# samkatt/fba-pomdp

Measured on AMD Instinct MI355X. Metric: simulated env steps/sec (belief+rollout), higher is better.
Workload: dtype f64

## Files before the change

fba_pomdp_amd/csrc/fba_engine.hip:

```cpp
#include <hip/hip_runtime.h>

#include <algorithm>
#include <cmath>
#include <cstdarg>
#include <cstdio>
#include <cstdlib>
#include <cstring>
#include <string>
#include <map>
#include <memory>
#include <vector>

#include "fba_belief_factors.h"
#include "fba_launch_plan.h"
#include "fba_snapshot_format.h"

using namespace fba;

namespace {

thread_local std::string g_create_error;

struct EventPair {
    hipEvent_t a, b;
// ... 1151 lines not shown
{
    std::vector<unsigned long long> h((size_t)n);
    hipError_t e = hipMemcpy(h.data(), dev, h.size() * sizeof(unsigned long long), hipMemcpyDeviceToHost);
    if (e != hipSuccess) {
        *rc = fail(c, FBA_EHIP, "counter download failed: %s", hipGetErrorString(e));
        return 0;
    }
    uint64_t s = 0;
    for (auto v : h) s += v;
    return s;
}


struct CreateSwitches {
    bool double_buffer, node_visits, wide_hash, dense_particles;
    bool no_etiger, tiger_gather, no_compact;
    int hist_multi;
    bool hist_lockstep;
    bool tree_records, rows_hbm, stride_full;
    bool is_multi_min_set;
    int is_multi_min;
    int scratch_slots, node_bound;
    int node_words;
};
CreateSwitches read_create_switches()
{
    const auto number = [](const char* v, int unset) { return v ? std::atoi(v) : unset; };
    const auto says   = [](const char* v, const char* word) { return v && !std::strcmp(v, word); };
    const auto at_least = [](const char* v, int least) { return v ? std::max(least, std::atoi(v)) : 0; };
    CreateSwitches s{};
    s.double_buffer   = std::getenv("FBA_DOUBLE_BUFFER") != nullptr;
    s.node_visits     = std::getenv("FBA_NODE_VISITS") != nullptr;
    s.wide_hash       = std::getenv("FBA_WIDE_HASH") != nullptr;
    s.dense_particles = std::getenv("FBA_DENSE_PARTICLES") != nullptr;
    s.no_etiger       = number(std::getenv("FBA_NO_ETIGER"), 0) != 0;
    s.tiger_gather    = number(std::getenv("FBA_TIGER_GATHER"), 0) != 0;
    s.no_compact      = number(std::getenv("FBA_NO_COMPACT"), 0) != 0;
    const char* multi = std::getenv("FBA_HIST_MULTI");
    s.hist_multi      = multi ? (std::atoi(multi) != 0 ? 2 : 1) : 0;
    s.hist_lockstep   = number(std::getenv("FBA_HIST_LOCKSTEP"), 1) != 0;
    s.tree_records    = says(std::getenv("FBA_HIST_TREE"), "records");
    s.rows_hbm        = says(std::getenv("FBA_HIST_ROWS"), "hbm");
    s.stride_full     = says(std::getenv("FBA_HIST_STRIDE"), "full");
    const char* multi_min = std::getenv("FBA_IS_MULTI_MIN");
    s.is_multi_min_set = multi_min != nullptr;
    s.is_multi_min     = multi_min ? std::max(1, std::atoi(multi_min)) : IS_MAX_CHUNKS * 256 + 1;
    s.scratch_slots   = at_least(std::getenv("FBA_SCRATCH_SLOTS"), 1);
    s.node_bound      = at_least(std::getenv("FBA_NODE_BOUND"), 2);
    s.node_words      = number(std::getenv("FBA_NODE_WORDS"), 0);
    return s;
}

int check_arguments(const fba_config& cfg)
{
    if (cfg.sims < 1 && cfg.planner == FBA_PLANNER_POUCT) return fail(nullptr, FBA_EINVAL, "cannot initiate POUCT with %d simulations, must be greater than 0", cfg.sims);
    if (cfg.horizon <= 0) return fail(nullptr, FBA_EINVAL, "cannot initiate POUCT with %d horizon, must be greater than 0", cfg.horizon);
    if (cfg.horizon > 255) return fail(nullptr, FBA_EINVAL, "horizon %d exceeds the 255 steps a stream address holds", cfg.horizon);
    if (cfg.particles < 1) return fail(nullptr, FBA_EINVAL, "cannot initiate belief with n = %d", cfg.particles);
    if (cfg.discount <= 0 || cfg.discount > 1) return fail(nullptr, FBA_EINVAL, "discount must be in (0, 1]");
    if (cfg.runs < 1 || cfg.episodes < 1) return fail(nullptr, FBA_EINVAL, "runs and episodes must be >= 1");
    if (cfg.episodes > 65535) return fail(nullptr, FBA_EINVAL, "episodes %d exceeds the 65535 a stream address holds", cfg.episodes);
    if (cfg.model == FBA_MODEL_POMDP && cfg.episodes != 1) return fail(nullptr, FBA_EINVAL, "planning runs have exactly one episode per run");
    int ndev = 0;
    if (hipGetDeviceCount(&ndev) != hipSuccess || ndev <= 0) return fail(nullptr, FBA_ENODEVICE, "no HIP device visible: libfba_hip has no CPU path");
    if (cfg.device < 0 || cfg.device >= ndev) return fail(nullptr, FBA_EINVAL, "device %d out of range (%d visible)", cfg.device, ndev);
    return FBA_OK;
}

bool has_fully_connected_prior(const fba_config& cfg)
{
    return cfg.model == FBA_MODEL_BA_FACTORED && (dom_is_ftiger(cfg.domain) || is_ca(cfg.domain) || is_sys(cfg.domain)) &&
           !(is_ca(cfg.domain) && cfg.structure_prior == FBA_SP_FULLY_CONNECTED);
// ... 320 lines not shown
    }
    P.search_budget = (P.hist && P.hist != 3 && cfg.search_budget > 0) ? cfg.search_budget : 0;
    const size_t per_particle_aux = (P.hist && P.belief == FBA_BELIEF_REJECTION) ? 0 : (size_t)(2 * 8 + 8 + 4 * (MAXINC + 1));
    t.per_slot = (size_t)P.N * (per_particle_aux + ((P.reinvig || P.cheat) ? 4 : (P.incub ? 6 : (P.hist ? 1 : 2))) * (size_t)P.Cs * 4) +
                 (t.bkt_lines ? t.bkt_lines * 128 : (size_t)D.max_nodes * D.node_words * 4 + (size_t)t.hcap * t.hash_entry) + 1024;
    return FBA_OK;
}

int slot_count(const fba_config& cfg, const TreePlan& t, size_t budget)
{
    if (cfg.slots > 0) return cfg.slots;
    return std::min((int)std::min<size_t>(std::max<size_t>(budget / t.per_slot, 1), 32768), cfg.runs);
}

bool weighted_filters(const Problem& P) { return P.belief == FBA_BELIEF_IMPORTANCE || P.incub; }

int plan_filters(fba_ctx* c, const CreateSwitches& sw)
{
    const Problem& P = c->P;
    DeviceState& D = c->D;
    D.single_rec      = P.hist && !sw.double_buffer ? 1 : 0;
    D.ab_rows_hbm = sw.rows_hbm ? 1 : 0; D.ab_hist_multi = sw.hist_multi; D.ab_no_etiger = sw.no_etiger ? 1 : 0; D.ab_tiger_gather = sw.tiger_gather ? 1 : 0;
    D.ab_lockstep = sw.hist_lockstep ? 1 : 0;
    D.side_w = 1 + (P.model == FBA_MODEL_BA_FACTORED ? c->fdesc.FS + c->fdesc.FO : (P.model == FBA_MODEL_BA_TABLE ? 2 : 0));
    if (P.hist) D.side_w = 2;
    D.is_multi    = weighted_filters(P) && P.N >= sw.is_multi_min;
    D.ctot_stride = (P.N + 255) / 256 + 2;
    if (P.mh) {
        if (D.is_multi) return fail(c, FBA_EINVAL, "mh-within-gibbs belief: at most %d particles per slot", IS_MAX_CHUNKS * 256);
        if (c->fdesc.nvar > MH_MAXVAR) return fail(c, FBA_EINVAL, "mh beliefs: at most %d structure words per particle", MH_MAXVAR);
        size_t words = (size_t)3 * P.Cs + (size_t)P.S * P.A * P.S + (size_t)P.A * P.S * P.O + 2;
        words += 2 * ((size_t)(P.horizon + 1) * P.S + P.S) + (size_t)P.episodes * (P.horizon + 1) + 2 * (size_t)P.horizon + 2;
        D.mh_scratch_words = (int32_t)((words + 3) & ~(size_t)3);
    }
    if (P.cheat && D.is_multi) return fail(c, FBA_EINVAL, "cheating-reinvigoration belief: at most %d particles per slot", IS_MAX_CHUNKS * 256);
    return FBA_OK;
}

bool compact_filters_ok(const fba_ctx* c, const CreateSwitches& sw)
{
    const Problem& P = c->P;
    return c->cfg.domain == FBA_DOM_TIGER_EPISODIC && P.belief == FBA_BELIEF_REJECTION && !P.reinvig && !P.incub && !P.cheat && !P.nested &&
           !P.point && run_steps(c->cfg) <= 32767 && !sw.dense_particles && !sw.no_compact && P.search_budget <= 0 &&
           kernel_name(update_plan(P, c->D).filter) == K_REJECT_TIGER_ONCE && search_plan(P, c->D).kernel == SEARCH_READS_COMPACT;
}

// ... 2049 lines not shown
```

fba_pomdp_amd/csrc/fba_launch_plan.h:

```cpp
#pragma once

#include "fba_kernels.h"

namespace fba {

__host__ __device__ __forceinline__ bool root_children_in_lds(const Problem& P, const DeviceState& D)
{
    return P.A * P.O <= ROOT_CHILDREN && D.max_nodes <= 32767;
}
constexpr int ET_NODE_WORDS = 9;
__host__ __device__ __forceinline__ size_t search_lds_words(const Problem& P, const DeviceState& D, bool stage, bool etiger)
{
    const int depth_cap = P.max_depth > 0 ? P.max_depth : 1;
    if (etiger)
        return (size_t)((depth_cap + 1) / 2) * SEARCH_BLOCK + (stage ? (size_t)P.Cs * SEARCH_BLOCK : 0) + (size_t)2 * ET_NODE_WORDS * SEARCH_BLOCK;
    return (size_t)depth_cap * SEARCH_BLOCK * 2 + (stage ? (size_t)P.Cs * SEARCH_BLOCK : 0) +
           (root_children_in_lds(P, D) ? (size_t)P.A * P.O * SEARCH_BLOCK / 2 : 0);
}
constexpr int HIST_TREES = SEARCH_BLOCK / HIST_QUAD;
constexpr int H2_WAVES = 4;
__host__ __device__ __forceinline__ size_t h2_shared_bytes(const Problem& P, bool lrows)
{
    const int K = hist_row_width(P.hist_row);
    return lrows ? (size_t)P.hist_rid_bytes + (size_t)P.hist_distinct * K * sizeof(float) : (size_t)4 * HistLayout(P.gw_N, P.gw_G, 4).ostride * sizeof(float);
// ... 42 lines not shown
}
constexpr uint32_t importance_key(bool reg, int tiger_table, bool hist, bool wlds) { return kernel_key(K_IMPORTANCE, reg, tiger_table, hist, wlds); }
constexpr bool tiger_filter_in_lds(uint32_t key)
{
    return kernel_name(key) == K_REJECT_TIGER_LDS || kernel_name(key) == K_REJECT_TIGER_ONCE || kernel_name(key) == K_REJECT_TIGER_ONCE_GATHER;
}
constexpr bool reads_packed_tiger(uint32_t key)
{
    return key == search_key(true, 4, false, 2, FBA_MODEL_BA_TABLE) || key == SEARCH_READS_COMPACT || key == reject_key(false, 2, 0, 512) ||
           tiger_filter_in_lds(key) || key == importance_key(false, 2, false, false) || key == importance_key(false, 2, false, true);
}
constexpr bool reads_packed_ftiger(uint32_t key, int fs = 4)
{
    return key == reject_key(false, 0, fs, REJECT_BLOCK, true) || key == search_key(true, 4, false, 0, FBA_MODEL_BA_FACTORED, fs, false, true, false) ||
           key == search_key(true, 4, false, 0, FBA_MODEL_BA_FACTORED, fs, false, true, true) || (fs > 2 && reads_packed_ftiger(key, fs - 1));
}
constexpr bool updates_history_records(uint32_t key)
{
    return kernel_name(key) == K_REJECT_HIST || kernel_name(key) == K_REJECT_TAB_HIST || kernel_name(key) == K_IS_MULTI_TAB_STEP ||
           kernel_name(key) == K_IS_MULTI_CA_STEP || key == importance_key(false, 0, true, false) || key == importance_key(false, 0, true, true) ||
           (kernel_name(key) == K_IS_MULTI_STEP && (key >> 12 & 63));
}

struct SearchPlan {
    uint32_t kernel;
    int block, slots_per_block;
    size_t lds;
    int raise_lds;
    bool order_first;
    int grid(int slots) const { return (slots + slots_per_block - 1) / slots_per_block; }
};
inline SearchPlan search_plan(const Problem& P, const DeviceState& D)
{
    SearchPlan pl{0, SEARCH_BLOCK, SEARCH_BLOCK, 0, 0, false};
    const int depth_cap = P.max_depth > 0 ? P.max_depth : 1;
    if (P.hist == 3) {
        pl.kernel = kernel_key(K_SEARCH_CA_HIST, 4);
        pl.lds    = ca_hist_search_lds(P);
        return pl;
    }
    if (P.hist) {
        const int K = hist_row_width(P.hist_row);
        pl.slots_per_block = HIST_TREES;
        if (!D.bkt) {
            pl.kernel = kernel_key(K_SEARCH_HIST, K);
            pl.lds = (size_t)depth_cap * HIST_TREES * (sizeof(double) + sizeof(int32_t) + sizeof(float) + sizeof(int32_t)) + (size_t)P.Cs * HIST_TREES * sizeof(float);
            return pl;
        }
        const bool tab = P.hist == 2, flat = P.belief == FBA_BELIEF_REJECTION;
        const bool lrows = !tab && P.hist_lds != nullptr && !D.ab_rows_hbm;
        const size_t shared = tab ? 0 : h2_shared_bytes(P, lrows);
        int nw = H2_WAVES;
        while (nw > 1 && shared + (size_t)nw * h2_wave_bytes(P) > 64 * 1024) nw >>= 1;
        pl.lds = shared + (size_t)nw * h2_wave_bytes(P);
        pl.block = 64 * nw;
        pl.slots_per_block = HIST_TREES * nw;
        pl.raise_lds = pl.lds > 64 * 1024 ? (int)pl.lds : 0;
        pl.order_first = D.ab_lockstep != 0;
        pl.kernel = tab ? kernel_key(K_SEARCH_TABHIST, flat) : kernel_key(flat ? K_HIST2_FLAT_SEARCH : K_SEARCH_HIST2, K, lrows);
        return pl;
    }
    const bool stage = P.model != FBA_MODEL_POMDP && P.Cs <= SEARCH_STAGE_WORDS;
    const bool plain_tree  = P.planner == FBA_PLANNER_POUCT && !D.hash;
    const bool tiger_table = tiger_table_model(P) && stage && plain_tree;
    const bool tiger_pomdp = P.model == FBA_MODEL_POMDP && dom_is_tiger(P.domain) && plain_tree;
    const int fs           = ftiger_features(P);
    const bool ftiger      = fs >= 2 && fs <= 4 && plain_tree;
    const bool et = !D.ab_no_etiger && etiger_ok(P, D) && (tiger_table || tiger_pomdp || (ftiger && P.ft_packed));
    pl.lds = search_lds_words(P, D, stage, et) * sizeof(uint32_t);
    if (P.model == FBA_MODEL_BA_FACTORED && !ftiger)
        pl.lds = ((pl.lds + 15) & ~(size_t)15) + (((size_t)P.fd_bytes + 15) & ~(size_t)15);
    if (tiger_table) pl.kernel = search_key(true, 4, false, P.packed ? 2 : 1, FBA_MODEL_BA_TABLE, 0, false, false, et);
    else if (tiger_pomdp) pl.kernel = search_key(false, 4, false, 0, FBA_MODEL_POMDP, 0, true, false, et);
    else if (ftiger) pl.kernel = search_key(stage || P.ft_packed, 4, false, 0, FBA_MODEL_BA_FACTORED, fs, false, P.ft_packed != 0, et);
    else {
        const int amax  = P.A <= 4 ? 4 : (P.A <= 8 ? 8 : (P.A <= 16 ? 16 : 24));
        const int model = amax < 24 && (P.model == FBA_MODEL_BA_FACTORED || P.model == FBA_MODEL_BA_TABLE) ? P.model : FBA_MODEL_POMDP;
        pl.kernel = search_key(stage && model != FBA_MODEL_POMDP, amax, P.dirichlet_regular && model != FBA_MODEL_POMDP, 0, model);
    }
    return pl;
}

struct LaunchStep {
    uint32_t kernel;
    int block;
    int rows;
    int per_group;
    size_t lds;
    int raise_lds;
    int arg;
    bool chunked;
    bool shadow;
    dim3 grid(int slots) const { return rows ? dim3(rows, slots) : dim3((slots + per_group - 1) / per_group); }
};
struct LaunchPlan {
    LaunchStep step[12];
    int n = 0;
    uint32_t filter = 0;
    LaunchStep& add(uint32_t kernel, int block = 256, int rows = 0, int per_group = 1, size_t lds = 0, int arg = 0)
    {
        step[n] = LaunchStep{kernel, block, rows, per_group, lds, 0, arg, false, false};
        return step[n++];
// ... 117 lines not shown
```

fba_pomdp_amd/csrc/fba_search.hip:

```cpp
#include <algorithm>
#include <cstdio>
#include <cstdlib>
#include <cstring>

#include "fba_kernels_common.h"

namespace fba {

__device__ __forceinline__ int et_reward_code(double r) { return r == -1.0 ? 0 : (r == 10.0 ? 1 : 2); }
__device__ __forceinline__ double et_reward(int code) { return code == 0 ? -1.0 : (code == 1 ? 10.0 : -100.0); }
#ifdef FBA_PROFILE_SEARCH
__device__ unsigned long long g_search_prof[8];
#define PROF_MARK(r) { const long long now_ = clock64(); prof_[r] += now_ - prev_; prev_ = now_; }
#else
#define PROF_MARK(r)
#endif
template <bool STAGE, int AMAX, bool REG, int TIGER_TABLE, int MODEL, int FTIGER = 0, bool TIGER_POMDP = false, bool FTP = false, bool ETIGER = false>
__global__ void __launch_bounds__(SEARCH_BLOCK) search_kernel(Problem P, DeviceState D)
{
    if (TIGER_POMDP) {
        P.S = 2; P.A = 3; P.O = 2; P.C = 0; P.Cs = 4; P.planner = FBA_PLANNER_POUCT;
        if (P.domain != FBA_DOM_TIGER_CONTINUOUS) P.domain = FBA_DOM_TIGER_EPISODIC;
        P.belief = P.belief == FBA_BELIEF_IMPORTANCE ? FBA_BELIEF_IMPORTANCE : FBA_BELIEF_REJECTION;
        D.cn_off = 1; D.cq_off = 4; D.child_off = 10; D.node_words = 16; D.hash = nullptr;
    }
    P.model = MODEL;
    if (FTIGER > 0) {
        P.S = 1 << FTIGER; P.A = 3; P.O = 2;
        if (P.domain != FBA_DOM_FTIGER_CONTINUOUS) P.domain = FBA_DOM_FTIGER_EPISODIC;
        if (ETIGER) P.domain = FBA_DOM_FTIGER_EPISODIC;
    }
    if (ETIGER) { P.A = 3; P.O = 2; }
    if (TIGER_TABLE) {
        P.model = FBA_MODEL_BA_TABLE; P.planner = FBA_PLANNER_POUCT;
        P.S = 2; P.A = 3; P.O = 2; P.phi_len = 12; P.C = 24; P.Cs = 32;
// ... 55 lines not shown
    double r_cq[AMAX];
#pragma unroll
    for (int a = 0; a < AMAX; ++a) { r_cn[a] = 0; r_cq[a] = 0.0; }
    if (root_lds)
        for (int k = 0; k < P.A * P.O; ++k) rootch[k * SEARCH_BLOCK] = -1;
    uint32_t l1_exists = 0;
    int4 cy_h2 = make_int4(0, 0, 0, 0), cy_h3 = make_int4(0, 0, 0, 0);
    double cy_q2 = 0, cy_q3 = 0;
    int4* tab      = hash_table(D, e);
    const uint32_t epoch = D.hash ? hash_begin_search(D, e, tab, 0, 1) : 0;

    constexpr bool COMPACT = TIGER_TABLE == 2 && ETIGER;
    const int lazy_c = (slot_lazy(D, e) ? 1 : 0) | (COMPACT && D.compact[e] ? 2 : 0);
    if (COMPACT && (lazy_c & 2)) {
#pragma unroll
        for (int w = 0; w < 10; ++w)
            if (w != 2 && w != 5) stage[w * SEARCH_BLOCK] = 0.f;
    }
    int ts_src = -1, ts_state = 0;
    if (P.planner == FBA_PLANNER_TS) {
        g.stream(FBA_PHASE_SEARCH, (uint32_t)P.sims + 2u);
        ts_src = nested ? nested_sample(P, D, e, g, ts_state) : belief_sample_uniform(P, D, g);
    }
    int sim = 0, mode = 0;
    int s = 0, node = 0, dtg = 0, plen = 0, rdepth = 0;
    const float* cnt = prec;
    double rret = 0, rdisc = 1;
#ifdef FBA_PROFILE_SEARCH
    long long prof_[8] = {0, 0, 0, 0, 0, 0, 0, 0}, prev_ = clock64();
#endif
    while (true) {
        PROF_MARK(6)
        if (mode == 0) {
            if (sim >= P.sims) break;
            g.stream(FBA_PHASE_SEARCH, (uint32_t)sim);
            int nest_state = ts_state;
            const int src = ts_src >= 0 ? ts_src : (nested ? nested_sample(P, D, e, g, nest_state) : belief_sample_uniform(P, D, g));
            cnt = prec + (size_t)src * P.Cs;
            if (COMPACT && (lazy_c & 2)) {
                const uint4 v = reinterpret_cast<const uint4*>(prec)[src];
                stage[2 * SEARCH_BLOCK]  = __uint_as_float(v.x);
                stage[5 * SEARCH_BLOCK]  = __uint_as_float(v.y);
                stage[10 * SEARCH_BLOCK] = __uint_as_float(v.z);
                stage[11 * SEARCH_BLOCK] = __uint_as_float(v.w & 0x7fffffffu);
                s = (int)(v.w >> 31);
                stage[12 * SEARCH_BLOCK] = __int_as_float(s);
            } else if (STAGE) {
                const float4* rp = reinterpret_cast<const float4*>(cnt);
                const int n4 = (P.C + 4) >> 2;
                constexpr int NB = TIGER_TABLE == 2 ? 4 : 12;
                for (int k0 = 0; k0 < n4; k0 += NB) {
                    float4 v[NB];
#pragma unroll
                    for (int q = 0; q < NB; ++q) v[q] = rp[min(k0 + q, n4 - 1)];
#pragma unroll
                    for (int q = 0; q < NB; ++q) {
                        const int k = k0 + q;
                        if (k < n4) {
                            stage[(4 * k + 0) * SEARCH_BLOCK] = v[q].x;
                            stage[(4 * k + 1) * SEARCH_BLOCK] = v[q].y;
                            stage[(4 * k + 2) * SEARCH_BLOCK] = v[q].z;
                            stage[(4 * k + 3) * SEARCH_BLOCK] = v[q].w;
                        }
                    }
                }
                s = __float_as_int(stage[P.C * SEARCH_BLOCK]);
            } else {
                s = rec_state(cnt, P.C);
            }
            if (lazy_c & 1) s = lazy_state(P, g, src);
            if (nested) s = nest_state;
            node = 0; dtg = max_tree_depth; plen = 0; mode = 1;
        }
        PROF_MARK(0)
        bool finish = false, do_step = true;
        double delayed = 0;
        int a = 0;
        if (mode == 1) {
            tree_depth = max(tree_depth, max_tree_depth - dtg);
            if (dtg == 0) { finish = true; do_step = false; }
            else if (ETIGER) {
                int cn[AMAX], vis = r_vis;
                double cq[AMAX];
#pragma unroll
                for (int a2 = 0; a2 < AMAX; ++a2) { cn[a2] = r_cn[a2]; cq[a2] = r_cq[a2]; }
                if (node < 0) {
                    const uint32_t* nd = l1 + (size_t)(-1 - node) * ET_NODE_WORDS * SEARCH_BLOCK;
                    const uint32_t w0 = nd[0], w1 = nd[1 * SEARCH_BLOCK];
                    cn[0] = (int)(w0 & 0xffffu); cn[1] = (int)(w0 >> 16); cn[2] = (int)(w1 & 0xffffu);
#pragma unroll
                    for (int a2 = 0; a2 < 3; ++a2)
                        cq[a2] = __hiloint2double((int)nd[(4 + 2 * a2) * SEARCH_BLOCK], (int)nd[(3 + 2 * a2) * SEARCH_BLOCK]);
                    vis = (cn[0] + cn[1]) + cn[2];
                } else if (node > 0) {
                    const int32_t* rec = tree + (size_t)node * W;
                    const int4 h      = *reinterpret_cast<const int4*>(rec);
                    const double2 q01 = *reinterpret_cast<const double2*>(rec + 4);
                    const double q2   = *reinterpret_cast<const double*>(rec + 8);
                    vis = h.x; cn[0] = h.y; cn[1] = h.z; cn[2] = h.w;
                    cq[0] = q01.x; cq[1] = q01.y; cq[2] = q2;
                }
                a = ucb_pick<AMAX>(P, g, D.log1p_tab, vis, cn, cq, true);
                if (plen == 2) { cy_h2 = make_int4(vis, cn[0], cn[1], cn[2]); cy_q2 = a == 0 ? cq[0] : (a == 1 ? cq[1] : cq[2]); }
                if (plen == 3) { cy_h3 = make_int4(vis, cn[0], cn[1], cn[2]); cy_q3 = a == 0 ? cq[0] : (a == 1 ? cq[1] : cq[2]); }
            }
            else if (node == 0) a = ucb_pick<AMAX>(P, g, D.log1p_tab, r_vis, r_cn, r_cq, true);
            else a = ucb_select<AMAX>(P, D, g, tree + (size_t)node * W, true);
        } else {
            a = domain_random_action(P, g, s);
        }
        PROF_MARK(1)
        int o;
        double r;
        bool term;
        if (do_step) {
            if (FTIGER > 0 && STAGE && FTP)
                term = ftiger_step_packed<(FTIGER > 0 ? FTIGER : 1)>(P, g, LdsView<SEARCH_BLOCK>{stage}, s, a, o, r, NoInc{});
            else if (FTIGER > 0 && STAGE) term = ftiger_step<(FTIGER > 0 ? FTIGER : 1)>(P, g, LdsView<SEARCH_BLOCK>{stage}, s, a, o, r, NoInc{});
            else if (FTIGER > 0) term = ftiger_step<(FTIGER > 0 ? FTIGER : 1)>(P, g, GlobalSearchView{cnt}, s, a, o, r, NoInc{});
            else if (TIGER_TABLE == 2)
                term = tiger_step_packed(P, g, [&](int w) { return __float_as_uint(stage[w * SEARCH_BLOCK]); }, s_prior, s, a, o, r, NoInc{});
            else if (STAGE) term = sim_step<REG>(P, g, LdsView<SEARCH_BLOCK>{stage}, s, a, o, r, NoInc{});
            else term = sim_step<REG>(P, g, GlobalSearchView{cnt}, s, a, o, r, NoInc{});
            ++steps;
#ifdef FBA_PROFILE_SEARCH
        }
        PROF_MARK(2)
        if (do_step) {
#endif
            if (ETIGER && mode == 1) {
                path16[(size_t)plen * SEARCH_BLOCK] = (uint16_t)((node < 0 ? -1 - node : node) | (a << 12) | (et_reward_code(r) << 14));
                ++plen;
                if (term) finish = true;
                else {
                    int c = 0;
                    if (node == 0) c = ((l1_exists >> o) & 1u) ? -1 - o : 0;
                    else if (node < 0) {
                        const uint32_t w2 = l1[((size_t)(-1 - node) * ET_NODE_WORDS + 2) * SEARCH_BLOCK];
                        c = (int)(o ? (w2 >> 16) : (w2 & 0xffffu));
                    } else {
                        c = tree[(size_t)node * W + D.child_off + 2 * 2 + o];
                        c = c < 0 ? 0 : c;
                    }
                    if (c != 0) { node = c; --dtg; }
                    else {
                        const int nn = min(n_nodes, D.max_nodes - 1);
                        ++n_nodes;
                        if (node == 0) {
                            uint32_t* nd = l1 + (size_t)o * ET_NODE_WORDS * SEARCH_BLOCK;
#pragma unroll
                            for (int k = 0; k < ET_NODE_WORDS; ++k) nd[k * SEARCH_BLOCK] = 0;
                            l1_exists |= 1u << o;
                        } else {
                            node_init(D, tree + (size_t)nn * W, P.A, P.O);
                            if (node < 0) {
                                uint32_t* w2 = l1 + ((size_t)(-1 - node) * ET_NODE_WORDS + 2) * SEARCH_BLOCK;
                                *w2 = o ? ((*w2 & 0xffffu) | ((uint32_t)nn << 16)) : ((*w2 & 0xffff0000u) | (uint32_t)nn);
                            } else tree[(size_t)node * W + D.child_off + 2 * 2 + o] = nn;
                        }
                        mode = 2; rdepth = dtg - 1; rret = 0; rdisc = 1;
                        if (rdepth == 0) finish = true;
                    }
                }
            } else if (mode == 1) {
                path_r[(size_t)plen * SEARCH_BLOCK]  = (float)r;
                path_na[(size_t)plen * SEARCH_BLOCK] = (node << 5) | a  ;
                ++plen;
                if (term) finish = true;
                else {
                    const bool at_root_lds = root_lds && node == 0;
                    const int c = at_root_lds ? rootch[(a * P.O + o) * SEARCH_BLOCK] : child_get(P, D, tree, tab, epoch, node, a, o);
                    if (c >= 0) { node = c; --dtg; }
                    else {
                        const int nn = min(n_nodes, D.max_nodes - 1);
                        ++n_nodes;
                        node_init(D, tree + (size_t)nn * W, P.A, P.O);
                        if (at_root_lds) rootch[(a * P.O + o) * SEARCH_BLOCK] = (int16_t)nn;
                        else child_set(P, D, tree, tab, epoch, node, a, o, nn);
                        mode = 2; rdepth = dtg - 1; rret = 0; rdisc = 1;
                        if (rdepth == 0) finish = true;
                    }
                }
            } else {
                rret += r * rdisc;
                rdisc *= P.gamma;
                --rdepth;
                if (rdepth == 0 || term) { delayed = rret; finish = true; }
            }
        }
        PROF_MARK(3)
        if (finish) {
            double del = delayed;
            for (int k = plen - 1; k >= (ETIGER ? 4 : 1); --k) {
                const int na     = ETIGER ? (int)path16[(size_t)k * SEARCH_BLOCK] : path_na[(size_t)k * SEARCH_BLOCK];
                const double ret = (ETIGER ? et_reward(na >> 14) : (double)path_r[(size_t)k * SEARCH_BLOCK]) + P.gamma * del;
                const int act    = ETIGER ? ((na >> 12) & 3) : (na & 31);
                int32_t* rec = tree + (size_t)(ETIGER ? (na & 0xfff) : (na >> 5)) * W;
                double* q    = reinterpret_cast<double*>(rec + D.cq_off) + act;
                int n;
                if (P.A == 3) {
                    int4* hp = reinterpret_cast<int4*>(rec);
                    int4 h   = *hp;
                    n = act == 0 ? ++h.y : (act == 1 ? ++h.z : ++h.w);
                    ++h.x;
                    *hp = h;
                } else {
                    n = ++rec[D.cn_off + act];
                    if (D.cn_off) ++rec[0];
                }
                *q += (ret - *q) / (double)n;
                del = ret;
            }
            if (ETIGER) {
#pragma unroll
                for (int lv = 3; lv >= 2; --lv)
// ... 23 lines not shown
                uint32_t* qw     = nd + (size_t)(3 + 2 * act) * SEARCH_BLOCK;
                double q         = __hiloint2double((int)qw[SEARCH_BLOCK], (int)qw[0]);
                q += (ret - q) / (double)n;
                qw[0]            = (uint32_t)__double2loint(q);
                qw[SEARCH_BLOCK] = (uint32_t)__double2hiint(q);
                del = ret;
            }
            if (plen > 0) {
                const double ret = (ETIGER ? et_reward((int)path16[0] >> 14) : (double)path_r[0]) + P.gamma * del;
                const int act    = ETIGER ? (((int)path16[0] >> 12) & 3) : (path_na[0] & 31);
                int n = 0;
                double q = 0.0;
#pragma unroll
                for (int a2 = 0; a2 < AMAX; ++a2)
                    if (a2 == act) { n = r_cn[a2]; q = r_cq[a2]; }
                ++n;
                q += (ret - q) / (double)n;
#pragma unroll
                for (int a2 = 0; a2 < AMAX; ++a2)
                    if (a2 == act) { r_cn[a2] = n; r_cq[a2] = q; }
                ++r_vis;
            }
            ++sim;
            mode = 0;
        }
        PROF_MARK(4)
#ifdef FBA_PROFILE_SEARCH
        prof_[5] += 1;
#endif
    }
#ifdef FBA_PROFILE_SEARCH
    if (lane == 0)
        for (int r = 0; r < 8; ++r) atomicAdd(&g_search_prof[r], (unsigned long long)prof_[r]);
#endif
    g.stream(FBA_PHASE_SEARCH, (uint32_t)P.sims + 1u);
    if (n_nodes > D.max_nodes) atomicCAS(D.fault, 0, -(1 + e));
    const int best = ucb_pick<AMAX>(P, g, D.log1p_tab, 0, r_cn, r_cq, false);
    D.action[e]    = best;
    D.sim_steps[e] += steps;
    fba_trace_rec& rec = D.cur[e];
    rec.n_nodes    = n_nodes;
    rec.tree_depth = tree_depth;
#pragma unroll
    for (int a = 0; a < FBA_MAX_ACTIONS; ++a) {
        rec.root_n[a] = a < AMAX && a < P.A ? r_cn[a < AMAX ? a : 0] : 0;
        rec.root_q[a] = a < AMAX && a < P.A ? r_cq[a < AMAX ? a : 0] : 0.0;
    }
}

template <int K>
__global__ void __launch_bounds__(SEARCH_BLOCK) search_hist_kernel(Problem P, DeviceState D)
{
    constexpr int AMAX = 4;
    P.model = FBA_MODEL_BA_FACTORED; P.domain = FBA_DOM_GRIDWORLD; P.A = 4; P.belief = FBA_BELIEF_IMPORTANCE;
    extern __shared__ double lds[];
    const int lane = threadIdx.x, tl = lane >> 2;
// ... 472 lines not shown
                for (int a2 = 0; a2 < AMAX; ++a2)
                    if (a2 == act) { r_cn[a2] = nv; r_cq[a2] = q; }
                ++r_vis;
            }
            ++sim;
            mode = 0;
        }
    }
    g.stream(FBA_PHASE_SEARCH, (uint32_t)P.sims + 1u);
    if (n_nodes > D.max_nodes) atomicCAS(D.fault, 0, -(1 + e));
    const int best = ucb_pick<AMAX>(P, g, D.log1p_tab, 0, r_cn, r_cq, false);
    D.action[e]    = best;
    D.sim_steps[e] += steps;
    fba_trace_rec& rec = D.cur[e];
    rec.n_nodes    = n_nodes;
    rec.tree_depth = tree_depth;
#pragma unroll
    for (int a = 0; a < FBA_MAX_ACTIONS; ++a) {
        rec.root_n[a] = a < AMAX && a < P.A ? r_cn[a < AMAX ? a : 0] : 0;
        rec.root_q[a] = a < AMAX && a < P.A ? r_cq[a < AMAX ? a : 0] : 0.0;
    }
}

void launch_search(const Problem& P, const DeviceState& D, hipStream_t st)
{
    const SearchPlan pl = search_plan(P, D);
    static const size_t lds_pad = std::getenv("FBA_SEARCH_LDS_PAD") ? (size_t)std::atoi(std::getenv("FBA_SEARCH_LDS_PAD")) : 0;
    const size_t lds = pl.lds + (kernel_name(pl.kernel) == K_SEARCH ? lds_pad : 0);
    const dim3 grid(pl.grid(P.E)), block(pl.block);
    if (pl.order_first) hipLaunchKernelGGL(search_order_kernel, dim3(1), dim3(1024), 0, st, P, D);
#define FBA_LAUNCH(...)                                                                                                                     \
    {                                                                                                                                       \
        if (pl.raise_lds) (void)hipFuncSetAttribute(reinterpret_cast<const void*>(&__VA_ARGS__), hipFuncAttributeMaxDynamicSharedMemorySize, pl.raise_lds); \
        hipLaunchKernelGGL((__VA_ARGS__), grid, block, lds, st, P, D);                                                                      \
        return;                                                                                                                             \
    }
#define FBA_SEARCH(...) case search_key(__VA_ARGS__): FBA_LAUNCH(search_kernel<__VA_ARGS__>)
#define FBA_HIST_SEARCH(NAME, KERNEL, ...) case kernel_key(NAME, __VA_ARGS__): FBA_LAUNCH(KERNEL<__VA_ARGS__>)
    switch (pl.kernel) {
        FBA_HIST_SEARCH(K_SEARCH_CA_HIST, search_ca_hist_kernel, 4)
        FBA_HIST_SEARCH(K_SEARCH_TABHIST, search_tabhist_kernel, true)
        FBA_HIST_SEARCH(K_SEARCH_TABHIST, search_tabhist_kernel, false)
        FBA_HIST_SEARCH(K_HIST2_FLAT_SEARCH, hist2_flat_search, 8, true)
        FBA_HIST_SEARCH(K_HIST2_FLAT_SEARCH, hist2_flat_search, 8, false)
        FBA_HIST_SEARCH(K_HIST2_FLAT_SEARCH, hist2_flat_search, 12, true)
        FBA_HIST_SEARCH(K_HIST2_FLAT_SEARCH, hist2_flat_search, 12, false)
        FBA_HIST_SEARCH(K_HIST2_FLAT_SEARCH, hist2_flat_search, 16, true)
        FBA_HIST_SEARCH(K_HIST2_FLAT_SEARCH, hist2_flat_search, 16, false)
        FBA_HIST_SEARCH(K_SEARCH_HIST2, search_hist2_kernel, 8, true)
// ... 41 lines not shown
        FBA_SEARCH(false, 8, true, 0, FBA_MODEL_BA_TABLE)
        FBA_SEARCH(false, 8, false, 0, FBA_MODEL_BA_TABLE)
        FBA_SEARCH(false, 8, false, 0, FBA_MODEL_POMDP)
        FBA_SEARCH(true, 16, true, 0, FBA_MODEL_BA_FACTORED)
        FBA_SEARCH(true, 16, false, 0, FBA_MODEL_BA_FACTORED)
        FBA_SEARCH(true, 16, true, 0, FBA_MODEL_BA_TABLE)
        FBA_SEARCH(true, 16, false, 0, FBA_MODEL_BA_TABLE)
        FBA_SEARCH(false, 16, true, 0, FBA_MODEL_BA_FACTORED)
        FBA_SEARCH(false, 16, false, 0, FBA_MODEL_BA_FACTORED)
        FBA_SEARCH(false, 16, true, 0, FBA_MODEL_BA_TABLE)
        FBA_SEARCH(false, 16, false, 0, FBA_MODEL_BA_TABLE)
        FBA_SEARCH(false, 16, false, 0, FBA_MODEL_POMDP)
        FBA_SEARCH(false, 24, false, 0, FBA_MODEL_POMDP)
    }
#undef FBA_HIST_SEARCH
#undef FBA_SEARCH
#undef FBA_LAUNCH
    std::fprintf(stderr, "launch_search: no instantiation behind kernel key %#x\n", pl.kernel);
    std::abort();
}
#ifdef FBA_PROFILE_SEARCH
extern "C" int fba_debug_search_profile(unsigned long long* out, int reset)
{
    if (hipMemcpyFromSymbol(out, HIP_SYMBOL(g_search_prof), sizeof(unsigned long long) * 8) != hipSuccess) return -1;
    if (reset) {
        const unsigned long long z[8] = {0, 0, 0, 0, 0, 0, 0, 0};
        if (hipMemcpyToSymbol(HIP_SYMBOL(g_search_prof), z, sizeof z) != hipSuccess) return -1;
    }
    return 0;
}
#endif

}
```

fba_pomdp_amd/csrc/fba_state.h:

```cpp
#pragma once

#include <stdint.h>

#include "fba_device.h"

namespace fba {

struct DeviceState {
    int32_t* run;
    int32_t* episode;
    int32_t* t;
    uint8_t* active;
    uint8_t* need_update;
    uint8_t* need_reset;
    uint8_t* need_init;
    uint8_t* adv;
    int32_t* env_state;
    double* ret;
    double* disc;
    int32_t* action;
    int32_t* obs;
    uint8_t* bufsel;
    double* p_weight;
    float* p_rec;
// ... 4 lines not shown
    uint8_t* compact;
    int8_t compact_on;
    unsigned long long* upd_compact_full;
    unsigned long long* upd_compact;
    int32_t* fault;
    uint8_t* cheat_pending;
    int16_t* mh_a;
    int16_t* mh_o;
    int32_t* mh_ep_len;
    int32_t* mh_n_ep;
    float* rec_scratch;
    uint8_t* copy_pending;
    int32_t single_rec;
    int32_t* rec_buf;
    int32_t slot_base;
    int32_t scratch_slots;
    int32_t* slot_list;
    int32_t* list_count;
    int32_t* list_count_host;
    int8_t ab_rows_hbm;
    int8_t ab_hist_multi;
    int8_t ab_no_etiger;
    int8_t ab_tiger_gather;
    int8_t ab_lockstep;
    int32_t* search_order;
    int32_t* scratch_idx;
    int32_t use_list;
    float* p_rec_sh;
    double* p_weight_sh;
    uint8_t* bufsel_sh;
    uint8_t* need_update_sh;
    const int32_t* inc_order;
    int32_t shadow;
    int32_t* nest_s;
    int32_t* nest_sel;
    double* nest_scan;
    double* nest_total;
    float* mh_scratch;
    int32_t mh_scratch_words;
    int32_t* p_side;
    uint32_t* hist_cnt;
    int32_t side_w;
    double* wscan;
    double* ctot;
    double* is_tot;
    int32_t ctot_stride;
// ... 44 lines not shown
```

Measured before the change: 48.81 billion.

## Restart MCTS simulations in warp-wide quorum batches to reduce divergence

Restructures the per-lane search loop so finished lanes wait idle until a quorum fraction of the wavefront has finished. The waiting lanes then run backup and sample a new particle together, instead of each lane doing so as soon as it finishes. This is meant to cut divergent execution of the expensive backup and staging code paths. The cost is idle lanes during the wait. The quorum defaults to 60/64 for two compact kernel keys and to full lockstep (64) otherwise, and can be overridden through an environment variable.

```diff
diff --git a/fba_pomdp_amd/csrc/fba_engine.hip b/fba_pomdp_amd/csrc/fba_engine.hip
--- a/fba_pomdp_amd/csrc/fba_engine.hip
+++ b/fba_pomdp_amd/csrc/fba_engine.hip
@@ -1197,6 +1197,7 @@
     int is_multi_min;
     int scratch_slots, node_bound;
     int node_words;
+    int search_quorum;
 };
 CreateSwitches read_create_switches()
 {
@@ -1223,6 +1224,7 @@
     s.scratch_slots   = at_least(std::getenv("FBA_SCRATCH_SLOTS"), 1);
     s.node_bound      = at_least(std::getenv("FBA_NODE_BOUND"), 2);
     s.node_words      = number(std::getenv("FBA_NODE_WORDS"), 0);
+    s.search_quorum   = search_quorum_switch(std::getenv("FBA_SEARCH_QUORUM"));
     return s;
 }
 
@@ -1589,6 +1591,7 @@
     D.single_rec      = P.hist && !sw.double_buffer ? 1 : 0;
     D.ab_rows_hbm = sw.rows_hbm ? 1 : 0; D.ab_hist_multi = sw.hist_multi; D.ab_no_etiger = sw.no_etiger ? 1 : 0; D.ab_tiger_gather = sw.tiger_gather ? 1 : 0;
     D.ab_lockstep = sw.hist_lockstep ? 1 : 0;
+    D.search_quorum = (int8_t)sw.search_quorum;
     D.side_w = 1 + (P.model == FBA_MODEL_BA_FACTORED ? c->fdesc.FS + c->fdesc.FO : (P.model == FBA_MODEL_BA_TABLE ? 2 : 0));
     if (P.hist) D.side_w = 2;
     D.is_multi    = weighted_filters(P) && P.N >= sw.is_multi_min;
diff --git a/fba_pomdp_amd/csrc/fba_launch_plan.h b/fba_pomdp_amd/csrc/fba_launch_plan.h
--- a/fba_pomdp_amd/csrc/fba_launch_plan.h
+++ b/fba_pomdp_amd/csrc/fba_launch_plan.h
@@ -1,4 +1,6 @@
 #pragma once
+
+#include <cstdlib>
 
 #include "fba_kernels.h"
 
@@ -88,17 +90,29 @@
            (kernel_name(key) == K_IS_MULTI_STEP && (key >> 12 & 63));
 }
 
+constexpr int SEARCH_QUORUM_LOCKSTEP = 64;
+constexpr uint32_t SEARCH_C3 = search_key(true, 4, false, 0, FBA_MODEL_BA_FACTORED, 3, false, true, true);
+constexpr int search_quorum_default(uint32_t kernel)
+{
+    return kernel == SEARCH_READS_COMPACT  || kernel == SEARCH_C3 ? 60 : SEARCH_QUORUM_LOCKSTEP;
+}
+inline int search_quorum_switch(const char* text)
+{
+    const int v = text ? std::atoi(text) : 0;
+    return v >= 1 && v <= SEARCH_QUORUM_LOCKSTEP ? v : 0;
+}
 struct SearchPlan {
     uint32_t kernel;
     int block, slots_per_block;
     size_t lds;
     int raise_lds;
     bool order_first;
+    int quorum;
     int grid(int slots) const { return (slots + slots_per_block - 1) / slots_per_block; }
 };
 inline SearchPlan search_plan(const Problem& P, const DeviceState& D)
 {
-    SearchPlan pl{0, SEARCH_BLOCK, SEARCH_BLOCK, 0, 0, false};
+    SearchPlan pl{0, SEARCH_BLOCK, SEARCH_BLOCK, 0, 0, false, SEARCH_QUORUM_LOCKSTEP};
     const int depth_cap = P.max_depth > 0 ? P.max_depth : 1;
     if (P.hist == 3) {
         pl.kernel = kernel_key(K_SEARCH_CA_HIST, 4);
@@ -144,6 +158,7 @@
         const int model = amax < 24 && (P.model == FBA_MODEL_BA_FACTORED || P.model == FBA_MODEL_BA_TABLE) ? P.model : FBA_MODEL_POMDP;
         pl.kernel = search_key(stage && model != FBA_MODEL_POMDP, amax, P.dirichlet_regular && model != FBA_MODEL_POMDP, 0, model);
     }
+    pl.quorum = D.search_quorum >= 1 && D.search_quorum <= SEARCH_QUORUM_LOCKSTEP ? D.search_quorum : search_quorum_default(pl.kernel);
     return pl;
 }
 
diff --git a/fba_pomdp_amd/csrc/fba_search.hip b/fba_pomdp_amd/csrc/fba_search.hip
--- a/fba_pomdp_amd/csrc/fba_search.hip
+++ b/fba_pomdp_amd/csrc/fba_search.hip
@@ -10,7 +10,7 @@
 __device__ __forceinline__ int et_reward_code(double r) { return r == -1.0 ? 0 : (r == 10.0 ? 1 : 2); }
 __device__ __forceinline__ double et_reward(int code) { return code == 0 ? -1.0 : (code == 1 ? 10.0 : -100.0); }
 #ifdef FBA_PROFILE_SEARCH
-__device__ unsigned long long g_search_prof[8];
+__device__ unsigned long long g_search_prof[12];
 #define PROF_MARK(r) { const long long now_ = clock64(); prof_[r] += now_ - prev_; prev_ = now_; }
 #else
 #define PROF_MARK(r)
@@ -112,175 +112,26 @@
         g.stream(FBA_PHASE_SEARCH, (uint32_t)P.sims + 2u);
         ts_src = nested ? nested_sample(P, D, e, g, ts_state) : belief_sample_uniform(P, D, g);
     }
-    int sim = 0, mode = 0;
+    int sim = -1, mode = 0;
     int s = 0, node = 0, dtg = 0, plen = 0, rdepth = 0;
     const float* cnt = prec;
     double rret = 0, rdisc = 1;
-#ifdef FBA_PROFILE_SEARCH
-    long long prof_[8] = {0, 0, 0, 0, 0, 0, 0, 0}, prev_ = clock64();
+    const int quorum = D.search_quorum;
+#ifdef FBA_PROFILE_SEARCH
+    long long prof_[12] = {0, 0, 0, 0, 0, 0, 0, 0, 0, 0, 0, 0}, prev_ = clock64();
 #endif
     while (true) {
         PROF_MARK(6)
-        if (mode == 0) {
-            if (sim >= P.sims) break;
-            g.stream(FBA_PHASE_SEARCH, (uint32_t)sim);
-            int nest_state = ts_state;
-            const int src = ts_src >= 0 ? ts_src : (nested ? nested_sample(P, D, e, g, nest_state) : belief_sample_uniform(P, D, g));
-            cnt = prec + (size_t)src * P.Cs;
-            if (COMPACT && (lazy_c & 2)) {
-                const uint4 v = reinterpret_cast<const uint4*>(prec)[src];
-                stage[2 * SEARCH_BLOCK]  = __uint_as_float(v.x);
-                stage[5 * SEARCH_BLOCK]  = __uint_as_float(v.y);
-                stage[10 * SEARCH_BLOCK] = __uint_as_float(v.z);
-                stage[11 * SEARCH_BLOCK] = __uint_as_float(v.w & 0x7fffffffu);
-                s = (int)(v.w >> 31);
-                stage[12 * SEARCH_BLOCK] = __int_as_float(s);
-            } else if (STAGE) {
-                const float4* rp = reinterpret_cast<const float4*>(cnt);
-                const int n4 = (P.C + 4) >> 2;
-                constexpr int NB = TIGER_TABLE == 2 ? 4 : 12;
-                for (int k0 = 0; k0 < n4; k0 += NB) {
-                    float4 v[NB];
-#pragma unroll
-                    for (int q = 0; q < NB; ++q) v[q] = rp[min(k0 + q, n4 - 1)];
-#pragma unroll
-                    for (int q = 0; q < NB; ++q) {
-                        const int k = k0 + q;
-                        if (k < n4) {
-                            stage[(4 * k + 0) * SEARCH_BLOCK] = v[q].x;
-                            stage[(4 * k + 1) * SEARCH_BLOCK] = v[q].y;
-                            stage[(4 * k + 2) * SEARCH_BLOCK] = v[q].z;
-                            stage[(4 * k + 3) * SEARCH_BLOCK] = v[q].w;
-                        }
-                    }
-                }
-                s = __float_as_int(stage[P.C * SEARCH_BLOCK]);
-            } else {
-                s = rec_state(cnt, P.C);
-            }
-            if (lazy_c & 1) s = lazy_state(P, g, src);
-            if (nested) s = nest_state;
-            node = 0; dtg = max_tree_depth; plen = 0; mode = 1;
-        }
-        PROF_MARK(0)
-        bool finish = false, do_step = true;
-        double delayed = 0;
-        int a = 0;
-        if (mode == 1) {
-            tree_depth = max(tree_depth, max_tree_depth - dtg);
-            if (dtg == 0) { finish = true; do_step = false; }
-            else if (ETIGER) {
-                int cn[AMAX], vis = r_vis;
-                double cq[AMAX];
-#pragma unroll
-                for (int a2 = 0; a2 < AMAX; ++a2) { cn[a2] = r_cn[a2]; cq[a2] = r_cq[a2]; }
-                if (node < 0) {
-                    const uint32_t* nd = l1 + (size_t)(-1 - node) * ET_NODE_WORDS * SEARCH_BLOCK;
-                    const uint32_t w0 = nd[0], w1 = nd[1 * SEARCH_BLOCK];
-                    cn[0] = (int)(w0 & 0xffffu); cn[1] = (int)(w0 >> 16); cn[2] = (int)(w1 & 0xffffu);
-#pragma unroll
-                    for (int a2 = 0; a2 < 3; ++a2)
-                        cq[a2] = __hiloint2double((int)nd[(4 + 2 * a2) * SEARCH_BLOCK], (int)nd[(3 + 2 * a2) * SEARCH_BLOCK]);
-                    vis = (cn[0] + cn[1]) + cn[2];
-                } else if (node > 0) {
-                    const int32_t* rec = tree + (size_t)node * W;
-                    const int4 h      = *reinterpret_cast<const int4*>(rec);
-                    const double2 q01 = *reinterpret_cast<const double2*>(rec + 4);
-                    const double q2   = *reinterpret_cast<const double*>(rec + 8);
-                    vis = h.x; cn[0] = h.y; cn[1] = h.z; cn[2] = h.w;
-                    cq[0] = q01.x; cq[1] = q01.y; cq[2] = q2;
-                }
-                a = ucb_pick<AMAX>(P, g, D.log1p_tab, vis, cn, cq, true);
-                if (plen == 2) { cy_h2 = make_int4(vis, cn[0], cn[1], cn[2]); cy_q2 = a == 0 ? cq[0] : (a == 1 ? cq[1] : cq[2]); }
-                if (plen == 3) { cy_h3 = make_int4(vis, cn[0], cn[1], cn[2]); cy_q3 = a == 0 ? cq[0] : (a == 1 ? cq[1] : cq[2]); }
-            }
-            else if (node == 0) a = ucb_pick<AMAX>(P, g, D.log1p_tab, r_vis, r_cn, r_cq, true);
-            else a = ucb_select<AMAX>(P, D, g, tree + (size_t)node * W, true);
-        } else {
-            a = domain_random_action(P, g, s);
-        }
-        PROF_MARK(1)
-        int o;
-        double r;
-        bool term;
-        if (do_step) {
-            if (FTIGER > 0 && STAGE && FTP)
-                term = ftiger_step_packed<(FTIGER > 0 ? FTIGER : 1)>(P, g, LdsView<SEARCH_BLOCK>{stage}, s, a, o, r, NoInc{});
-            else if (FTIGER > 0 && STAGE) term = ftiger_step<(FTIGER > 0 ? FTIGER : 1)>(P, g, LdsView<SEARCH_BLOCK>{stage}, s, a, o, r, NoInc{});
-            else if (FTIGER > 0) term = ftiger_step<(FTIGER > 0 ? FTIGER : 1)>(P, g, GlobalSearchView{cnt}, s, a, o, r, NoInc{});
-            else if (TIGER_TABLE == 2)
-                term = tiger_step_packed(P, g, [&](int w) { return __float_as_uint(stage[w * SEARCH_BLOCK]); }, s_prior, s, a, o, r, NoInc{});
-            else if (STAGE) term = sim_step<REG>(P, g, LdsView<SEARCH_BLOCK>{stage}, s, a, o, r, NoInc{});
-            else term = sim_step<REG>(P, g, GlobalSearchView{cnt}, s, a, o, r, NoInc{});
-            ++steps;
-#ifdef FBA_PROFILE_SEARCH
-        }
-        PROF_MARK(2)
-        if (do_step) {
-#endif
-            if (ETIGER && mode == 1) {
-                path16[(size_t)plen * SEARCH_BLOCK] = (uint16_t)((node < 0 ? -1 - node : node) | (a << 12) | (et_reward_code(r) << 14));
-                ++plen;
-                if (term) finish = true;
-                else {
-                    int c = 0;
-                    if (node == 0) c = ((l1_exists >> o) & 1u) ? -1 - o : 0;
-                    else if (node < 0) {
-                        const uint32_t w2 = l1[((size_t)(-1 - node) * ET_NODE_WORDS + 2) * SEARCH_BLOCK];
-                        c = (int)(o ? (w2 >> 16) : (w2 & 0xffffu));
-                    } else {
-                        c = tree[(size_t)node * W + D.child_off + 2 * 2 + o];
-                        c = c < 0 ? 0 : c;
-                    }
-                    if (c != 0) { node = c; --dtg; }
-                    else {
-                        const int nn = min(n_nodes, D.max_nodes - 1);
-                        ++n_nodes;
-                        if (node == 0) {
-                            uint32_t* nd = l1 + (size_t)o * ET_NODE_WORDS * SEARCH_BLOCK;
-#pragma unroll
-                            for (int k = 0; k < ET_NODE_WORDS; ++k) nd[k * SEARCH_BLOCK] = 0;
-                            l1_exists |= 1u << o;
-                        } else {
-                            node_init(D, tree + (size_t)nn * W, P.A, P.O);
-                            if (node < 0) {
-                                uint32_t* w2 = l1 + ((size_t)(-1 - node) * ET_NODE_WORDS + 2) * SEARCH_BLOCK;
-                                *w2 = o ? ((*w2 & 0xffffu) | ((uint32_t)nn << 16)) : ((*w2 & 0xffff0000u) | (uint32_t)nn);
-                            } else tree[(size_t)node * W + D.child_off + 2 * 2 + o] = nn;
-                        }
-                        mode = 2; rdepth = dtg - 1; rret = 0; rdisc = 1;
-                        if (rdepth == 0) finish = true;
-                    }
-                }
-            } else if (mode == 1) {
-                path_r[(size_t)plen * SEARCH_BLOCK]  = (float)r;
-                path_na[(size_t)plen * SEARCH_BLOCK] = (node << 5) | a  ;
-                ++plen;
-                if (term) finish = true;
-                else {
-                    const bool at_root_lds = root_lds && node == 0;
-                    const int c = at_root_lds ? rootch[(a * P.O + o) * SEARCH_BLOCK] : child_get(P, D, tree, tab, epoch, node, a, o);
-                    if (c >= 0) { node = c; --dtg; }
-                    else {
-                        const int nn = min(n_nodes, D.max_nodes - 1);
-                        ++n_nodes;
-                        node_init(D, tree + (size_t)nn * W, P.A, P.O);
-                        if (at_root_lds) rootch[(a * P.O + o) * SEARCH_BLOCK] = (int16_t)nn;
-                        else child_set(P, D, tree, tab, epoch, node, a, o, nn);
-                        mode = 2; rdepth = dtg - 1; rret = 0; rdisc = 1;
-                        if (rdepth == 0) finish = true;
-                    }
-                }
-            } else {
-                rret += r * rdisc;
-                rdisc *= P.gamma;
-                --rdepth;
-                if (rdepth == 0 || term) { delayed = rret; finish = true; }
-            }
-        }
-        PROF_MARK(3)
-        if (finish) {
-            double del = delayed;
+        const bool waiting = mode == 0 && sim < P.sims;
+        const int n_wait = __popcll(__ballot(waiting)), n_act = __popcll(__ballot(mode != 0));
+        if (n_wait + n_act == 0) break;
+        const bool boundary = n_act == 0 || n_wait * 64 >= quorum * (n_wait + n_act);
+#ifdef FBA_PROFILE_SEARCH
+        const bool lead_ = lane == __ffsll((unsigned long long)__ballot(true)) - 1;
+        if (lead_) { prof_[5] += 1; if (boundary) { prof_[9] += 1; prof_[10] += n_wait; } }
+#endif
+        if (boundary && waiting) {
+            double del = rret;
             for (int k = plen - 1; k >= (ETIGER ? 4 : 1); --k) {
                 const int na     = ETIGER ? (int)path16[(size_t)k * SEARCH_BLOCK] : path_na[(size_t)k * SEARCH_BLOCK];
                 const double ret = (ETIGER ? et_reward(na >> 14) : (double)path_r[(size_t)k * SEARCH_BLOCK]) + P.gamma * del;
@@ -350,16 +201,177 @@
                 ++r_vis;
             }
             ++sim;
-            mode = 0;
+            plen = 0;
         }
         PROF_MARK(4)
-#ifdef FBA_PROFILE_SEARCH
-        prof_[5] += 1;
-#endif
-    }
-#ifdef FBA_PROFILE_SEARCH
-    if (lane == 0)
-        for (int r = 0; r < 8; ++r) atomicAdd(&g_search_prof[r], (unsigned long long)prof_[r]);
+        if (boundary && waiting && sim < P.sims) {
+            g.stream(FBA_PHASE_SEARCH, (uint32_t)sim);
+            int nest_state = ts_state;
+            const int src = ts_src >= 0 ? ts_src : (nested ? nested_sample(P, D, e, g, nest_state) : belief_sample_uniform(P, D, g));
+            cnt = prec + (size_t)src * P.Cs;
+            if (COMPACT && (lazy_c & 2)) {
+                const uint4 v = reinterpret_cast<const uint4*>(prec)[src];
+                stage[2 * SEARCH_BLOCK]  = __uint_as_float(v.x);
+                stage[5 * SEARCH_BLOCK]  = __uint_as_float(v.y);
+                stage[10 * SEARCH_BLOCK] = __uint_as_float(v.z);
+                stage[11 * SEARCH_BLOCK] = __uint_as_float(v.w & 0x7fffffffu);
+                s = (int)(v.w >> 31);
+                stage[12 * SEARCH_BLOCK] = __int_as_float(s);
+            } else if (STAGE) {
+                const float4* rp = reinterpret_cast<const float4*>(cnt);
+                const int n4 = (P.C + 4) >> 2;
+                constexpr int NB = TIGER_TABLE == 2 ? 4 : 12;
+                for (int k0 = 0; k0 < n4; k0 += NB) {
+                    float4 v[NB];
+#pragma unroll
+                    for (int q = 0; q < NB; ++q) v[q] = rp[min(k0 + q, n4 - 1)];
+#pragma unroll
+                    for (int q = 0; q < NB; ++q) {
+                        const int k = k0 + q;
+                        if (k < n4) {
+                            stage[(4 * k + 0) * SEARCH_BLOCK] = v[q].x;
+                            stage[(4 * k + 1) * SEARCH_BLOCK] = v[q].y;
+                            stage[(4 * k + 2) * SEARCH_BLOCK] = v[q].z;
+                            stage[(4 * k + 3) * SEARCH_BLOCK] = v[q].w;
+                        }
+                    }
+                }
+                s = __float_as_int(stage[P.C * SEARCH_BLOCK]);
+            } else {
+                s = rec_state(cnt, P.C);
+            }
+            if (lazy_c & 1) s = lazy_state(P, g, src);
+            if (nested) s = nest_state;
+            node = 0; dtg = max_tree_depth; plen = 0; mode = 1;
+        }
+        PROF_MARK(0)
+        bool finish = false, do_step = mode != 0;
+        double delayed = 0;
+        int a = 0;
+        if (mode == 1) {
+            tree_depth = max(tree_depth, max_tree_depth - dtg);
+            if (dtg == 0) { finish = true; do_step = false; }
+            else if (ETIGER) {
+                int cn[AMAX], vis = r_vis;
+                double cq[AMAX];
+#pragma unroll
+                for (int a2 = 0; a2 < AMAX; ++a2) { cn[a2] = r_cn[a2]; cq[a2] = r_cq[a2]; }
+                if (node < 0) {
+                    const uint32_t* nd = l1 + (size_t)(-1 - node) * ET_NODE_WORDS * SEARCH_BLOCK;
+                    const uint32_t w0 = nd[0], w1 = nd[1 * SEARCH_BLOCK];
+                    cn[0] = (int)(w0 & 0xffffu); cn[1] = (int)(w0 >> 16); cn[2] = (int)(w1 & 0xffffu);
+#pragma unroll
+                    for (int a2 = 0; a2 < 3; ++a2)
+                        cq[a2] = __hiloint2double((int)nd[(4 + 2 * a2) * SEARCH_BLOCK], (int)nd[(3 + 2 * a2) * SEARCH_BLOCK]);
+                    vis = (cn[0] + cn[1]) + cn[2];
+                } else if (node > 0) {
+                    const int32_t* rec = tree + (size_t)node * W;
+                    const int4 h      = *reinterpret_cast<const int4*>(rec);
+                    const double2 q01 = *reinterpret_cast<const double2*>(rec + 4);
+                    const double q2   = *reinterpret_cast<const double*>(rec + 8);
+                    vis = h.x; cn[0] = h.y; cn[1] = h.z; cn[2] = h.w;
+                    cq[0] = q01.x; cq[1] = q01.y; cq[2] = q2;
+                }
+                a = ucb_pick<AMAX>(P, g, D.log1p_tab, vis, cn, cq, true);
+                if (plen == 2) { cy_h2 = make_int4(vis, cn[0], cn[1], cn[2]); cy_q2 = a == 0 ? cq[0] : (a == 1 ? cq[1] : cq[2]); }
+                if (plen == 3) { cy_h3 = make_int4(vis, cn[0], cn[1], cn[2]); cy_q3 = a == 0 ? cq[0] : (a == 1 ? cq[1] : cq[2]); }
+            }
+            else if (node == 0) a = ucb_pick<AMAX>(P, g, D.log1p_tab, r_vis, r_cn, r_cq, true);
+            else a = ucb_select<AMAX>(P, D, g, tree + (size_t)node * W, true);
+        } else if (mode == 2) {
+            a = domain_random_action(P, g, s);
+        }
+        PROF_MARK(1)
+        int o;
+        double r;
+        bool term;
+        if (do_step) {
+            if (FTIGER > 0 && STAGE && FTP)
+                term = ftiger_step_packed<(FTIGER > 0 ? FTIGER : 1)>(P, g, LdsView<SEARCH_BLOCK>{stage}, s, a, o, r, NoInc{});
+            else if (FTIGER > 0 && STAGE) term = ftiger_step<(FTIGER > 0 ? FTIGER : 1)>(P, g, LdsView<SEARCH_BLOCK>{stage}, s, a, o, r, NoInc{});
+            else if (FTIGER > 0) term = ftiger_step<(FTIGER > 0 ? FTIGER : 1)>(P, g, GlobalSearchView{cnt}, s, a, o, r, NoInc{});
+            else if (TIGER_TABLE == 2)
+                term = tiger_step_packed(P, g, [&](int w) { return __float_as_uint(stage[w * SEARCH_BLOCK]); }, s_prior, s, a, o, r, NoInc{});
+            else if (STAGE) term = sim_step<REG>(P, g, LdsView<SEARCH_BLOCK>{stage}, s, a, o, r, NoInc{});
+            else term = sim_step<REG>(P, g, GlobalSearchView{cnt}, s, a, o, r, NoInc{});
+            ++steps;
+#ifdef FBA_PROFILE_SEARCH
+        }
+        PROF_MARK(2)
+        if (do_step) {
+#endif
+            if (ETIGER && mode == 1) {
+                path16[(size_t)plen * SEARCH_BLOCK] = (uint16_t)((node < 0 ? -1 - node : node) | (a << 12) | (et_reward_code(r) << 14));
+                ++plen;
+                if (term) finish = true;
+                else {
+                    int c = 0;
+                    if (node == 0) c = ((l1_exists >> o) & 1u) ? -1 - o : 0;
+                    else if (node < 0) {
+                        const uint32_t w2 = l1[((size_t)(-1 - node) * ET_NODE_WORDS + 2) * SEARCH_BLOCK];
+                        c = (int)(o ? (w2 >> 16) : (w2 & 0xffffu));
+                    } else {
+                        c = tree[(size_t)node * W + D.child_off + 2 * 2 + o];
+                        c = c < 0 ? 0 : c;
+                    }
+                    if (c != 0) { node = c; --dtg; }
+                    else {
+                        const int nn = min(n_nodes, D.max_nodes - 1);
+                        ++n_nodes;
+                        if (node == 0) {
+                            uint32_t* nd = l1 + (size_t)o * ET_NODE_WORDS * SEARCH_BLOCK;
+#pragma unroll
+                            for (int k = 0; k < ET_NODE_WORDS; ++k) nd[k * SEARCH_BLOCK] = 0;
+                            l1_exists |= 1u << o;
+                        } else {
+                            node_init(D, tree + (size_t)nn * W, P.A, P.O);
+                            if (node < 0) {
+                                uint32_t* w2 = l1 + ((size_t)(-1 - node) * ET_NODE_WORDS + 2) * SEARCH_BLOCK;
+                                *w2 = o ? ((*w2 & 0xffffu) | ((uint32_t)nn << 16)) : ((*w2 & 0xffff0000u) | (uint32_t)nn);
+                            } else tree[(size_t)node * W + D.child_off + 2 * 2 + o] = nn;
+                        }
+                        mode = 2; rdepth = dtg - 1; rret = 0; rdisc = 1;
+                        if (rdepth == 0) finish = true;
+                    }
+                }
+            } else if (mode == 1) {
+                path_r[(size_t)plen * SEARCH_BLOCK]  = (float)r;
+                path_na[(size_t)plen * SEARCH_BLOCK] = (node << 5) | a  ;
+                ++plen;
+                if (term) finish = true;
+                else {
+                    const bool at_root_lds = root_lds && node == 0;
+                    const int c = at_root_lds ? rootch[(a * P.O + o) * SEARCH_BLOCK] : child_get(P, D, tree, tab, epoch, node, a, o);
+                    if (c >= 0) { node = c; --dtg; }
+                    else {
+                        const int nn = min(n_nodes, D.max_nodes - 1);
+                        ++n_nodes;
+                        node_init(D, tree + (size_t)nn * W, P.A, P.O);
+                        if (at_root_lds) rootch[(a * P.O + o) * SEARCH_BLOCK] = (int16_t)nn;
+                        else child_set(P, D, tree, tab, epoch, node, a, o, nn);
+                        mode = 2; rdepth = dtg - 1; rret = 0; rdisc = 1;
+                        if (rdepth == 0) finish = true;
+                    }
+                }
+            } else {
+                rret += r * rdisc;
+                rdisc *= P.gamma;
+                --rdepth;
+                if (rdepth == 0 || term) { delayed = rret; finish = true; }
+            }
+        }
+        PROF_MARK(3)
+        if (finish) { rret = delayed; mode = 0; }
+#ifdef FBA_PROFILE_SEARCH
+        {
+            const int n_step_ = __popcll(__ballot(do_step));
+            if (lead_) prof_[8] += n_step_;
+        }
+#endif
+    }
+#ifdef FBA_PROFILE_SEARCH
+    for (int r = 0; r < 12; ++r)
+        if ((r == 5 || r >= 8 ? prof_[r] != 0 : lane == 0) && r != 7 && r != 11) atomicAdd(&g_search_prof[r], (unsigned long long)prof_[r]);
 #endif
     g.stream(FBA_PHASE_SEARCH, (uint32_t)P.sims + 1u);
     if (n_nodes > D.max_nodes) atomicCAS(D.fault, 0, -(1 + e));
@@ -878,9 +890,11 @@
     }
 }
 
-void launch_search(const Problem& P, const DeviceState& D, hipStream_t st)
-{
-    const SearchPlan pl = search_plan(P, D);
+void launch_search(const Problem& P, const DeviceState& D0, hipStream_t st)
+{
+    const SearchPlan pl = search_plan(P, D0);
+    DeviceState D = D0;
+    D.search_quorum = (int8_t)pl.quorum;
     static const size_t lds_pad = std::getenv("FBA_SEARCH_LDS_PAD") ? (size_t)std::atoi(std::getenv("FBA_SEARCH_LDS_PAD")) : 0;
     const size_t lds = pl.lds + (kernel_name(pl.kernel) == K_SEARCH ? lds_pad : 0);
     const dim3 grid(pl.grid(P.E)), block(pl.block);
@@ -968,9 +982,9 @@
 #ifdef FBA_PROFILE_SEARCH
 extern "C" int fba_debug_search_profile(unsigned long long* out, int reset)
 {
-    if (hipMemcpyFromSymbol(out, HIP_SYMBOL(g_search_prof), sizeof(unsigned long long) * 8) != hipSuccess) return -1;
+    if (hipMemcpyFromSymbol(out, HIP_SYMBOL(g_search_prof), sizeof(unsigned long long) * 12) != hipSuccess) return -1;
     if (reset) {
-        const unsigned long long z[8] = {0, 0, 0, 0, 0, 0, 0, 0};
+        const unsigned long long z[12] = {0, 0, 0, 0, 0, 0, 0, 0, 0, 0, 0, 0};
         if (hipMemcpyToSymbol(HIP_SYMBOL(g_search_prof), z, sizeof z) != hipSuccess) return -1;
     }
     return 0;
diff --git a/fba_pomdp_amd/csrc/fba_state.h b/fba_pomdp_amd/csrc/fba_state.h
--- a/fba_pomdp_amd/csrc/fba_state.h
+++ b/fba_pomdp_amd/csrc/fba_state.h
@@ -50,6 +50,7 @@
     int8_t ab_hist_multi;
     int8_t ab_no_etiger;
     int8_t ab_tiger_gather;
+    int8_t search_quorum;
     int8_t ab_lockstep;
     int32_t* search_order;
     int32_t* scratch_idx;
```

After: 50.18 billion (median of 6 runs). +2.8%, better.
